# sedaprotocol/bn254

Hardware: AMD Instinct MI355X
Metric: BN254 pairings/sec (batch verify) (higher is better)
Workload: dtype u32

## Files before the change

bn254_amd/csrc/bn254_keydedup.hip:

```cpp
#include <hip/hip_runtime.h>

#define BN_SPLIT_FP2 1
#define bn254 bn254_kd
#include "bn254_pairing.h"
#include "bn254_keydedup.h"

using namespace bn254;

#include "bn254_ws.h"

#define KD_WG 256
#define KERNEL_KD_PAIR __global__ __launch_bounds__(KD_WG) __attribute__((amdgpu_waves_per_eu(2, 2)))
#define KERNEL_KD __global__ __launch_bounds__(KD_WG)
#define KERNEL_KD_CHAIN __global__ __launch_bounds__(BN_WAVE) __attribute__((amdgpu_waves_per_eu(1, 1)))

__device__ __forceinline__ uint32_t kd_hash(const uint32_t* w, uint32_t hash_mask) {
  uint32_t h = 0x9E3779B9u;
#pragma unroll
  for (int k = 0; k < 32; ++k) {
    h ^= w[k];
    h *= 0x85EBCA6Bu;
    h ^= h >> 13;
  }
  h ^= h >> 16; h *= 0xC2B2AE35u; h ^= h >> 16;
  return h & hash_mask;
}
__device__ __forceinline__ bool kd_same_key(const uint32_t* pks, uint32_t other, const uint32_t* w) {
  const uint32_t* o = pks + (size_t)other * 32;
  bool eq = true;
#pragma unroll
  for (int k = 0; k < 32; ++k) eq = eq && o[k] == w[k];
  return eq;
}
KERNEL_KD void k_kd_insert(const uint8_t* pks8, size_t n, KeyDedup kd) {
  const size_t i = (size_t)blockIdx.x * KD_WG + threadIdx.x;
  if (i >= n) return;
  const uint32_t* pks = (const uint32_t*)pks8;
  uint32_t w[32];
#pragma unroll
  for (int k = 0; k < 32; ++k) w[k] = pks[i * 32 + k];
  const uint32_t h = kd_hash(w, kd.hash_mask);
  for (uint32_t probe = 0; probe < KD_MAX_PROBES; ++probe) {
    const uint32_t s = (h + probe) & kd.slot_mask;
    uint32_t cur = __atomic_load_n(&kd.table[s], __ATOMIC_RELAXED);
    if (cur == KD_EMPTY) {
      cur = atomicCAS(&kd.table[s], KD_EMPTY, (uint32_t)i);
      if (cur == KD_EMPTY) {
        const uint32_t id = atomicAdd(&kd.ctl[KD_CTL_D], 1u);
        kd.slot_id[s] = id;
        if (id < kd.max_keys) kd.rep[id] = (uint32_t)i;
        kd.slot_of[i] = s;
        return;
      }
    }
    if (kd_same_key(pks, cur, w)) { kd.slot_of[i] = s; return; }
  }
  kd.slot_of[i] = KD_EMPTY;
  atomicOr(&kd.ctl[KD_CTL_FLAGS], (uint32_t)KD_OVERFLOW);
}
KERNEL_KD void k_kd_resolve(size_t n, KeyDedup kd) {
  const size_t i = (size_t)blockIdx.x * KD_WG + threadIdx.x;
  if (i >= n) return;
  const uint32_t s = kd.slot_of[i];
  kd.key_idx[i] = s == KD_EMPTY ? 0u : kd.slot_id[s];
}
__device__ __forceinline__ bool kd_viable(const KeyDedup& kd, size_t n) {
  const uint32_t d = kd.ctl[KD_CTL_D];
  return d <= kd.max_keys && (size_t)d * kd.min_mult <= n && (kd.ctl[KD_CTL_FLAGS] & KD_OVERFLOW) == 0;
}

__device__ __forceinline__ void kd_store_own(int32_t* dst, const Fp2& x) {
#pragma unroll
  for (int k = 0; k < BN_LIMBS; ++k) dst[(threadIdx.x & 1u) * BN_LIMBS + k] = x.c[0].v[k];
}
__device__ __forceinline__ Fp2 kd_load_own(const int32_t* src) {
  Fp2 r;
#pragma unroll
  for (int k = 0; k < BN_LIMBS; ++k) r.c[0].v[k] = src[(threadIdx.x & 1u) * BN_LIMBS + k];
  return r;
}
KERNEL_KD_CHAIN void k_kd_lines(const uint8_t* pks, size_t n, uint32_t flags, KeyDedup kd) {
  if (!kd_viable(kd, n)) return;
  const uint32_t j = (uint32_t)(((size_t)blockIdx.x * BN_WAVE + threadIdx.x) >> 1);
  if (j >= kd.ctl[KD_CTL_D]) return;
  __builtin_amdgcn_s_setprio(3);
  G2Affine q;
  const uint8_t st = decode_g2_pair_role(q, pks + 128 * (size_t)kd.rep[j], flags);
  const bool real = st == ST_OK && !q.inf;
  if (!real) { q.x = fp2_load_const(C_G2_GEN[0]); q.y = fp2_load_const(C_G2_GEN[1]); }
  if ((threadIdx.x & 1u) == 0) { kd.st[j] = st; kd.inf[j] = q.inf; }
  int32_t* rows = kd.lines + (size_t)j * BN_N_FIXED_LINES * BN_KEY_LINE_WORDS;
  int32_t* c2s = kd.c2 + (size_t)j * BN_N_FIXED_LINES * 2 * BN_LIMBS;
  const bool degenerate = kd_walk_raw_lines(q, [&](int idx, const Fp2& c0, const Fp2& c1, const Fp2& c2) {
    kd_store_own(c2s + (size_t)idx * 2 * BN_LIMBS, c2);
    kd_store_own(rows + (size_t)idx * BN_KEY_LINE_WORDS, c0);
    kd_store_own(rows + (size_t)idx * BN_KEY_LINE_WORDS + 2 * BN_LIMBS, c1);
  });
  if (real && degenerate && (threadIdx.x & 1u) == 0) atomicOr(&kd.ctl[KD_CTL_FLAGS], (uint32_t)KD_DEGENERATE);
}
KERNEL_KD_PAIR void k_kd_scale(size_t n, KeyDedup kd) {
  if (!kd_viable(kd, n)) return;
  const size_t p = ((size_t)blockIdx.x * KD_WG + threadIdx.x) >> 1;
  const uint32_t j = (uint32_t)(p / BN_N_FIXED_LINES), idx = (uint32_t)(p % BN_N_FIXED_LINES);
  if (j >= kd.ctl[KD_CTL_D]) return;
  int32_t* row = kd.lines + ((size_t)j * BN_N_FIXED_LINES + idx) * BN_KEY_LINE_WORDS;
  Fp2 r0, r1;
  kd_scale_line(kd_load_own(row), kd_load_own(row + 2 * BN_LIMBS), kd_load_own(kd.c2 + ((size_t)j * BN_N_FIXED_LINES + idx) * 2 * BN_LIMBS), r0, r1);
  kd_store_own(row, r0);
  kd_store_own(row + 2 * BN_LIMBS, r1);
}
KERNEL_KD void k_kd_decide(size_t n, KeyDedup kd, int force_generic) {
  if (threadIdx.x != 0) return;
  const bool keyed = !force_generic && kd_viable(kd, n) && (kd.ctl[KD_CTL_FLAGS] & KD_DEGENERATE) == 0;
  kd.ctl[KD_CTL_KEYED_N] = keyed ? (uint32_t)n : 0u;
  kd.ctl[KD_CTL_GENERIC_N] = keyed ? 0u : (uint32_t)n;
}

int bn254_kd_enqueue(const uint8_t* d_pks, size_t n, uint32_t flags, KeyDedup kd, int force_generic, hipStream_t s) {
  HIP_TRY(hipMemsetAsync(kd.table, 0xFF, ((size_t)kd.slot_mask + 1) * sizeof(uint32_t), s));
  HIP_TRY(hipMemsetAsync(kd.ctl, 0, KD_CTL_WORDS * sizeof(uint32_t), s));
  const unsigned g = (unsigned)((n + KD_WG - 1) / KD_WG);
  k_kd_insert<<<g, KD_WG, 0, s>>>(d_pks, n, kd);
  k_kd_resolve<<<g, KD_WG, 0, s>>>(n, kd);
  k_kd_lines<<<(unsigned)((2 * (size_t)kd.max_keys + BN_WAVE - 1) / BN_WAVE), BN_WAVE, 0, s>>>(d_pks, n, flags, kd);
  k_kd_scale<<<(unsigned)((2 * (size_t)kd.max_keys * BN_N_FIXED_LINES + KD_WG - 1) / KD_WG), KD_WG, 0, s>>>(n, kd);
  k_kd_decide<<<1, BN_WAVE, 0, s>>>(n, kd, force_generic);
  HIP_TRY(hipGetLastError());
  return 0;
}
```

Baseline: 14.34 million.

## Spread per-key Miller line generation across lane pairs via LDS line machine

Replaces the per-key serial line walk (one lane pair per key, 32 keys per wave) with an LDS-backed line machine where 9 lane pairs cooperatively execute each doubling/addition level for one key, 3 keys per wave. Each pair computes one product/linear op per level and a writer lane commits results to LDS, with wave fences between stages. This aims to cut the latency of the key-dedup line precompute for small numbers of distinct keys, at the cost of far fewer keys per wave, LDS traffic, and many barriers.

```diff
diff --git a/bn254_amd/csrc/bn254_kdlines.h b/bn254_amd/csrc/bn254_kdlines.h
--- /dev/null
+++ b/bn254_amd/csrc/bn254_kdlines.h
@@ -0,0 +1,78 @@
+#pragma once
+
+namespace bn254 {
+
+enum {
+  LS_KD_YQX = LS_LL0,
+  LS_KD_XQY = LS_LL1,
+  LS_KD_C1 = LS_LM0,
+  LS_KD_C2 = LS_LM1,
+  LS_KD_SLOTS = LS_REL0 + LS_REL_N
+};
+LM_TABLE LM_KD_ADD0[1][9] = {{
+    LM_E(lm_mul(LS_T1, LS_TQY, LS_TZ), lm_lin(LS_HOA, LS_TY, 1, LS_T1, -1)),
+    LM_E(lm_mul(LS_T2, LS_TQX, LS_TZ), lm_lin(LS_HOB, LS_TX, 1, LS_T2, -1)),
+    LM_E(lm_mul(LS_KD_YQX, LS_TY, LS_TQX), lm_lin(LS_KD_C2, LS_KD_YQX, 1, LS_KD_XQY, -1)),
+    LM_E(lm_mul(LS_KD_XQY, LS_TX, LS_TQY), lm_lin(LS_KD_C1, LS_T1, 1, LS_TY, -1)),
+    LM_E(LM_NOP_P, LM_NOP_L), LM_E(LM_NOP_P, LM_NOP_L), LM_E(LM_NOP_P, LM_NOP_L), LM_E(LM_NOP_P, LM_NOP_L), LM_E(LM_NOP_P, LM_NOP_L)}};
+
+enum KdLevel { KD_LV_INIT = 0, KD_LV_D0, KD_LV_D1, KD_LV_A0, KD_LV_A1, KD_LV_A2, KD_LV_N };
+enum { KD_LO_DBL = 0, KD_LO_ADD = 1 };
+BN_DEV int kd_line_slot(int kind, int coef) {
+  return kind == KD_LO_DBL ? (coef == 0 ? LS_HOA : coef == 1 ? LS_HOB : LS_HOC) : (coef == 0 ? LS_HOB : coef == 1 ? LS_KD_C1 : LS_KD_C2);
+}
+template <class Box> BN_DEV void kd_builder_init(Box& bx, const G2Affine& q) {
+  bx.put(bx.slot(LS_ONE), fp2_one()); bx.put(bx.slot(LS_B3), fp2_load_const(C_TWIST_3B));
+  bx.put(bx.slot(LS_PKX), q.x); bx.put(bx.slot(LS_PKY), q.y); bx.put(bx.slot(LS_CPKX), fp2_conj(q.x)); bx.put(bx.slot(LS_CPKY), fp2_conj(q.y));
+  bx.put(bx.slot(LS_FX1), fp2_load_const(C_TW_FROB_X1)); bx.put(bx.slot(LS_FY1), fp2_load_const(C_TW_FROB_Y1));
+  bx.put(bx.slot(LS_FX2), fp2_load_const(C_TW_FROB_X2));
+}
+template <class M> BN_DEV void kd_builder_program(M& m) {
+  m.level(KD_LV_INIT);
+  int idx = 0;
+#if defined(__HIPCC__)
+#pragma clang loop unroll(disable)
+#endif
+  for (int d = 0; d < 64; ++d) {
+    m.level(KD_LV_D0); m.level(KD_LV_D1); m.line(idx++, KD_LO_DBL);
+    const int digit = C_ATE_NAF[d];
+    if (digit != 0) {
+      m.add_point(LS_PKX, digit > 0 ? LS_PKY : LS_NPKY);
+      m.level(KD_LV_A0); m.level(KD_LV_A1); m.level(KD_LV_A2); m.line(idx++, KD_LO_ADD);
+    }
+  }
+  m.add_point(LS_Q1X, LS_Q1Y); m.level(KD_LV_A0); m.level(KD_LV_A1); m.level(KD_LV_A2); m.line(idx++, KD_LO_ADD);
+  m.add_point(LS_Q2X, LS_PKY); m.level(KD_LV_A0); m.level(KD_LV_A1); m.level(KD_LV_A2); m.line(idx++, KD_LO_ADD);
+}
+#if defined(__HIPCC__)
+__device__ __forceinline__ const LmEntry* kd_level_table(int lv) {
+  return lv == KD_LV_INIT ? LM_T_INIT[0] : lv == KD_LV_D0 ? LM_T_DBL[0] : lv == KD_LV_D1 ? LM_T_DBL[1] : lv == KD_LV_A0 ? LM_KD_ADD0[0]
+       : lv == KD_LV_A1 ? LM_T_ADD[1] : LM_T_ADD[2];
+}
+#else
+inline const LmEntry (&kd_level_table(int lv))[9] {
+  return lv == KD_LV_INIT ? LM_T_INIT[0] : lv == KD_LV_D0 ? LM_T_DBL[0] : lv == KD_LV_D1 ? LM_T_DBL[1] : lv == KD_LV_A0 ? LM_KD_ADD0[0]
+       : lv == KD_LV_A1 ? LM_T_ADD[1] : LM_T_ADD[2];
+}
+template <class Emit> bool kd_builder_model(const G2Affine& q, Emit&& emit) {
+  static LmHostBox bx;
+  for (int i = 0; i < LS_COUNT; ++i) bx.s[i] = fp2_zero();
+  kd_builder_init(bx, q);
+  struct M {
+    LmHostBox& bx;
+    Emit& emit;
+    bool degenerate;
+    void level(int lv) { lm_host_level(bx, kd_level_table(lv), 0, false, false); }
+    void add_point(int qx, int qy) { bx.s[LS_TQX] = bx.s[qx]; bx.s[LS_TQY] = bx.s[qy]; }
+    void line(int idx, int kind) {
+      const Fp2 c2 = bx.s[kd_line_slot(kind, 2)];
+      degenerate = fp2_is_zero(c2) || degenerate;
+      emit(idx, bx.s[kd_line_slot(kind, 0)], bx.s[kd_line_slot(kind, 1)], c2);
+    }
+  } m{bx, emit, false};
+  kd_builder_program(m);
+  return m.degenerate;
+}
+#endif
+
+}
diff --git a/bn254_amd/csrc/bn254_keydedup.hip b/bn254_amd/csrc/bn254_keydedup.hip
--- a/bn254_amd/csrc/bn254_keydedup.hip
+++ b/bn254_amd/csrc/bn254_keydedup.hip
@@ -4,6 +4,8 @@
 #define bn254 bn254_kd
 #include "bn254_pairing.h"
 #include "bn254_keydedup.h"
+#include "bn254_lmachine.h"
+#include "bn254_kdlines.h"
 
 using namespace bn254;
 
@@ -12,7 +14,6 @@
 #define KD_WG 256
 #define KERNEL_KD_PAIR __global__ __launch_bounds__(KD_WG) __attribute__((amdgpu_waves_per_eu(2, 2)))
 #define KERNEL_KD __global__ __launch_bounds__(KD_WG)
-#define KERNEL_KD_CHAIN __global__ __launch_bounds__(BN_WAVE) __attribute__((amdgpu_waves_per_eu(1, 1)))
 
 __device__ __forceinline__ uint32_t kd_hash(const uint32_t* w, uint32_t hash_mask) {
   uint32_t h = 0x9E3779B9u;
@@ -79,24 +80,99 @@
   for (int k = 0; k < BN_LIMBS; ++k) r.c[0].v[k] = src[(threadIdx.x & 1u) * BN_LIMBS + k];
   return r;
 }
-KERNEL_KD_CHAIN void k_kd_lines(const uint8_t* pks, size_t n, uint32_t flags, KeyDedup kd) {
+#define KD_LM_PER_WAVE 3
+#define KD_LM_LANES 18
+#define KD_LM_ROLE_STRIDE (LS_KD_SLOTS * BN_LIMBS + 1)
+#define KD_LM_KEY_STRIDE (2 * KD_LM_ROLE_STRIDE)
+#define KD_LM_LDS_WORDS (KD_LM_PER_WAVE * KD_LM_KEY_STRIDE)
+static_assert(KD_LM_PER_WAVE * KD_LM_LANES <= BN_WAVE, "keys per wave");
+#define KERNEL_KD_LM __global__ __launch_bounds__(BN_WAVE) __attribute__((amdgpu_waves_per_eu(1, 1)))
+#define KD_LM_FENCE() do { __builtin_amdgcn_fence(__ATOMIC_ACQ_REL, "wavefront"); __builtin_amdgcn_wave_barrier(); } while (0)
+
+extern __shared__ int32_t kd_lds[];
+
+struct KdLdsBox {
+  typedef unsigned Ref;
+  unsigned base;
+  __device__ __forceinline__ Ref slot(uint32_t id) const { return base + id * BN_LIMBS; }
+  __device__ __forceinline__ Fp2 get(Ref off) const {
+    Fp2 r;
+#pragma unroll
+    for (int i = 0; i < BN_LIMBS; ++i) r.c[0].v[i] = kd_lds[off + i];
+    return r;
+  }
+  __device__ __forceinline__ void put(Ref off, const Fp2& x) const {
+#pragma unroll
+    for (int i = 0; i < BN_LIMBS; ++i) kd_lds[off + i] = x.c[0].v[i];
+  }
+};
+struct KdLmDev {
+  KdLdsBox bx;
+  LmEntry e[KD_LV_N];
+  unsigned pair;
+  bool writer, live, degenerate;
+  int32_t* rows;
+  int32_t* c2s;
+  __device__ __forceinline__ void level(int lv) {
+    const LmEntry& en = e[lv];
+    {
+      const Fp2 pr = lm_stage_product(en, bx, 0);
+      KD_LM_FENCE();
+      if (writer && (en.w[1] & 255u) != (uint32_t)LS_DUMMY) bx.put(lm_product_out(en, bx, 0), pr);
+      KD_LM_FENCE();
+    }
+    const Fp2 li = lm_stage_linear(en, bx, 0, false, false);
+    KD_LM_FENCE();
+    if (writer && (en.w[4] & 255u) != (uint32_t)LS_DUMMY) bx.put(lm_linear_out(en, bx, 0), li);
+    KD_LM_FENCE();
+  }
+  __device__ __forceinline__ void add_point(int qx, int qy) {
+    const Fp2 x = bx.get(bx.slot((uint32_t)qx)), y = bx.get(bx.slot((uint32_t)qy));
+    if (writer) { bx.put(bx.slot(LS_TQX), x); bx.put(bx.slot(LS_TQY), y); }
+    KD_LM_FENCE();
+  }
+  __device__ __forceinline__ void line(int idx, int kind) {
+    degenerate = fp2_is_zero(bx.get(bx.slot((uint32_t)kd_line_slot(kind, 2)))) || degenerate;
+    const int c = pair < 3 ? (int)pair : 2;
+    const Fp2 v = bx.get(bx.slot((uint32_t)kd_line_slot(kind, c)));
+    if (live && pair < 3) kd_store_own(c == 2 ? c2s + (size_t)idx * 2 * BN_LIMBS : rows + (size_t)idx * BN_KEY_LINE_WORDS + (size_t)c * 2 * BN_LIMBS, v);
+  }
+};
+KERNEL_KD_LM void k_kd_lines(const uint8_t* pks, size_t n, uint32_t flags, KeyDedup kd) {
   if (!kd_viable(kd, n)) return;
-  const uint32_t j = (uint32_t)(((size_t)blockIdx.x * BN_WAVE + threadIdx.x) >> 1);
-  if (j >= kd.ctl[KD_CTL_D]) return;
+  const uint32_t d = kd.ctl[KD_CTL_D];
+  if ((uint32_t)blockIdx.x * KD_LM_PER_WAVE >= d) return;
   __builtin_amdgcn_s_setprio(3);
+  const unsigned l = threadIdx.x, v = l / KD_LM_LANES, role = l & 1u;
+  KdLmDev m;
+  m.writer = v < KD_LM_PER_WAVE;
+  const unsigned vslot = m.writer ? v : KD_LM_PER_WAVE - 1;
+  m.pair = (l % KD_LM_LANES) >> 1;
+  uint32_t j = (uint32_t)blockIdx.x * KD_LM_PER_WAVE + vslot;
+  m.live = m.writer && j < d;
+  if (j >= d) j = d - 1;
+  m.bx.base = vslot * KD_LM_KEY_STRIDE + role * KD_LM_ROLE_STRIDE;
   G2Affine q;
   const uint8_t st = decode_g2_pair_role(q, pks + 128 * (size_t)kd.rep[j], flags);
   const bool real = st == ST_OK && !q.inf;
   if (!real) { q.x = fp2_load_const(C_G2_GEN[0]); q.y = fp2_load_const(C_G2_GEN[1]); }
-  if ((threadIdx.x & 1u) == 0) { kd.st[j] = st; kd.inf[j] = q.inf; }
-  int32_t* rows = kd.lines + (size_t)j * BN_N_FIXED_LINES * BN_KEY_LINE_WORDS;
-  int32_t* c2s = kd.c2 + (size_t)j * BN_N_FIXED_LINES * 2 * BN_LIMBS;
-  const bool degenerate = kd_walk_raw_lines(q, [&](int idx, const Fp2& c0, const Fp2& c1, const Fp2& c2) {
-    kd_store_own(c2s + (size_t)idx * 2 * BN_LIMBS, c2);
-    kd_store_own(rows + (size_t)idx * BN_KEY_LINE_WORDS, c0);
-    kd_store_own(rows + (size_t)idx * BN_KEY_LINE_WORDS + 2 * BN_LIMBS, c1);
-  });
-  if (real && degenerate && (threadIdx.x & 1u) == 0) atomicOr(&kd.ctl[KD_CTL_FLAGS], (uint32_t)KD_DEGENERATE);
+  if (m.live && m.pair == 0 && role == 0) { kd.st[j] = st; kd.inf[j] = q.inf; }
+  if (m.writer) {
+    m.bx.put(m.bx.slot(LS_ZERO), fp2_zero()); m.bx.put(m.bx.slot(LS_DUMMY), fp2_zero());
+    kd_builder_init(m.bx, q);
+  }
+#pragma unroll
+  for (int lv = 0; lv < KD_LV_N; ++lv) {
+    const LmEntry* t = kd_level_table(lv);
+#pragma unroll
+    for (int k = 0; k < 5; ++k) m.e[lv].w[k] = t[m.pair].w[k];
+  }
+  m.rows = kd.lines + (size_t)j * BN_N_FIXED_LINES * BN_KEY_LINE_WORDS;
+  m.c2s = kd.c2 + (size_t)j * BN_N_FIXED_LINES * 2 * BN_LIMBS;
+  m.degenerate = false;
+  KD_LM_FENCE();
+  kd_builder_program(m);
+  if (m.live && real && m.degenerate && m.pair == 0 && role == 0) atomicOr(&kd.ctl[KD_CTL_FLAGS], (uint32_t)KD_DEGENERATE);
 }
 KERNEL_KD_PAIR void k_kd_scale(size_t n, KeyDedup kd) {
   if (!kd_viable(kd, n)) return;
@@ -122,7 +198,7 @@
   const unsigned g = (unsigned)((n + KD_WG - 1) / KD_WG);
   k_kd_insert<<<g, KD_WG, 0, s>>>(d_pks, n, kd);
   k_kd_resolve<<<g, KD_WG, 0, s>>>(n, kd);
-  k_kd_lines<<<(unsigned)((2 * (size_t)kd.max_keys + BN_WAVE - 1) / BN_WAVE), BN_WAVE, 0, s>>>(d_pks, n, flags, kd);
+  k_kd_lines<<<(unsigned)((kd.max_keys + KD_LM_PER_WAVE - 1) / KD_LM_PER_WAVE), BN_WAVE, KD_LM_LDS_WORDS * sizeof(int32_t), s>>>(d_pks, n, flags, kd);
   k_kd_scale<<<(unsigned)((2 * (size_t)kd.max_keys * BN_N_FIXED_LINES + KD_WG - 1) / KD_WG), KD_WG, 0, s>>>(n, kd);
   k_kd_decide<<<1, BN_WAVE, 0, s>>>(n, kd, force_generic);
   HIP_TRY(hipGetLastError());
```

Result: faster. 15.25 million, median of 6 (+6.3%).
